# vinodjanardhanan/BatchReactor.jl

Measured on AMD Instinct MI355X. Metric: reactor integrations/sec (CH4 GRI ensemble), higher is better.
Workload: dtype f64

## Files before the change

### batchreactor.jl_amd/_lib.py

```python
import ctypes as C
import os

import numpy as np

HERE = os.path.dirname(os.path.abspath(__file__))
LIBPATH = os.environ.get("BRHIP_LIB") or os.path.join(HERE, "libbrhip.so")

dp = C.POINTER(C.c_double)
ip = C.POINTER(C.c_int)


class MechDesc(C.Structure):
    _fields_ = [
        ("ng", C.c_int), ("ns", C.c_int), ("nrg", C.c_int), ("nrs", C.c_int),
        ("conv", C.c_int), ("p_std", C.c_double),
        ("molwt", dp), ("nasa", dp),
        ("g_nf", ip), ("g_nr", ip), ("g_f", ip), ("g_r", ip), ("g_rev", ip), ("g_tb", ip),
        ("g_arr", dp), ("g_low", dp), ("g_troe_n", ip), ("g_troe", dp), ("g_eff", dp),
        ("site_density", C.c_double), ("sigma", dp),
        ("s_nf", ip), ("s_np", ip), ("s_f", ip), ("s_p", ip), ("s_stick", ip), ("s_arr", dp),
        ("s_ncov", ip), ("s_cov_sp", ip), ("s_cov_eps", dp),
    ]


class Opts(C.Structure):
    _fields_ = [("rtol", C.c_double), ("atol", C.c_double), ("max_steps", C.c_int), ("device", C.c_int),
                ("hmax", C.c_double), ("trace_cap", C.c_int), ("unstable_factor", C.c_double),
                ("ignition_species", C.c_int), ("energy", C.c_int), ("T_end", dp), ("T_out", dp),
                ("nout", C.c_int), ("tout", dp), ("yout", dp),
                ("ntprog", C.c_int), ("tprog_t", dp), ("tprog_T", dp), ("ntprog_rows", C.c_int), ("tprog_row", ip),
                ("dq_jacobian", C.c_int), ("nmult", C.c_int), ("rate_mult", dp), ("rate_mult_row", ip),
                ("tout_per_reactor", C.c_int)]


NSTAT = 20
ENERGY_ADIABATIC_V = 1
BATCH_MAXCOMP = 64


class BatchInput(C.Structure):
    _fields_ = [("gas_mech", C.c_char * 256), ("surface_mech", C.c_char * 256), ("gasphase", C.c_char * 1024),
                ("T", C.c_double), ("p", C.c_double), ("Asv", C.c_double), ("time", C.c_double),
                ("has_T", C.c_int), ("has_p", C.c_int), ("has_Asv", C.c_int), ("has_time", C.c_int),
                ("ncomp", C.c_int), ("comp_is_mass", C.c_int),
                ("comp_names", (C.c_char * 32) * BATCH_MAXCOMP), ("comp_values", C.c_double * BATCH_MAXCOMP)]


EXPORTS = ["br_version", "br_last_error", "br_device_count", "br_mech_create", "br_mech_destroy", "br_mech_info", "br_mech_engine", "br_mech_launch_info",
           "br_rates", "br_rhs", "br_jacobian", "br_integrate", "br_integrate_traced", "br_integrate_multi", "br_integrate_dev",
           "br_last_kernel_ms", "br_debug_lu_solve", "br_mech_parse", "br_host_mech_desc", "br_host_mech_sizes",
           "br_host_mech_species", "br_host_mech_theta0", "br_host_mech_free", "br_mech_compile", "br_read_batch_xml",
           "br_integrate_host", "br_phase_tout_dev", "br_integrate_phase", "br_debug_group_eval",
           "br_debug_group_lu_solve", "br_sensitivity", "br_debug_tprog_eval", "br_debug_lane_eval",
           "br_debug_lane_lu_solve", "br_debug_wave_eval", "br_debug_energy_eval"]

RHS_FN = C.CFUNCTYPE(C.c_int, C.c_void_p, C.c_double, C.POINTER(C.c_double), C.POINTER(C.c_double))
STEP_FN = C.CFUNCTYPE(None, C.c_void_p, C.c_double, C.POINTER(C.c_double))

_lib = None


def lib():
    global _lib
    if _lib is not None:
        return _lib
    if not os.path.exists(LIBPATH):
        raise RuntimeError(f"libbrhip.so not built ({LIBPATH}); run __graft_entry__.build()")
    L = C.CDLL(LIBPATH)
    vp = C.c_void_p
    L.br_version.restype = C.c_int
    L.br_last_error.restype = C.c_char_p
    L.br_device_count.restype = C.c_int
    L.br_mech_create.argtypes = [C.POINTER(MechDesc), C.c_int, C.POINTER(vp)]
    L.br_mech_destroy.argtypes = [vp]
    L.br_mech_info.argtypes = [vp, ip, ip, ip, ip]
    L.br_mech_engine.argtypes = [vp]
    L.br_mech_engine.restype = C.c_int
    L.br_mech_launch_info.argtypes = [vp, ip, ip, C.POINTER(C.c_longlong)]
    L.br_rates.argtypes = [vp, C.c_int, dp, dp, dp, dp, dp, dp]
    L.br_rhs.argtypes = [vp, C.c_int, dp, dp, dp, dp]
    L.br_jacobian.argtypes = [vp, C.c_int, dp, dp, dp, dp]
    L.br_integrate.argtypes = [vp, C.c_int, dp, dp, dp, dp, C.POINTER(Opts), dp]
    L.br_integrate_traced.argtypes = [vp, C.c_int, dp, dp, dp, dp, C.POINTER(Opts), dp, dp]
    L.br_integrate_dev.argtypes = [vp, C.c_int, vp, vp, vp, vp, C.POINTER(Opts), vp, vp]
    L.br_integrate_multi.argtypes = [C.POINTER(vp), C.c_int, C.c_int, dp, dp, dp, dp, C.POINTER(Opts), dp]
    L.br_phase_tout_dev.argtypes = [C.c_int, vp, C.c_int, vp, vp, vp, vp]
    L.br_integrate_phase.argtypes = [vp, C.c_int, dp, dp, dp, dp, C.POINTER(Opts), dp, C.c_int, dp, dp, dp]
    L.br_sensitivity.argtypes = [vp, C.c_int, dp, dp, dp, dp, C.POINTER(Opts), C.c_double, C.c_int, ip, dp, dp, dp, dp,
                                 C.POINTER(C.c_longlong)]
    L.br_last_kernel_ms.argtypes = [vp, dp]
    L.br_debug_lu_solve.argtypes = [C.c_int, C.c_int, dp, dp, dp, dp, ip]
    L.br_debug_lu_solve.restype = C.c_int
    L.br_debug_group_eval.argtypes = [vp, C.c_int, dp, dp, dp, dp, dp]
    L.br_debug_group_eval.restype = C.c_int
    L.br_debug_group_lu_solve.argtypes = [C.c_int, C.c_int, C.c_int, C.c_int, dp, dp, dp, dp, ip, ip]
    L.br_debug_group_lu_solve.restype = C.c_int
    L.br_debug_tprog_eval.argtypes = [C.c_int, C.c_int, dp, dp, C.c_int, ip, C.c_int, dp, dp]
    L.br_debug_tprog_eval.restype = C.c_int
    L.br_debug_lane_eval.argtypes = [vp, C.c_int, dp, dp, C.c_int, dp, ip, dp, dp]
    L.br_debug_lane_eval.restype = C.c_int
    L.br_debug_lane_lu_solve.argtypes = [C.c_int, C.c_int, C.c_int, dp, dp, dp, ip, dp, ip, ip]
    L.br_debug_lane_lu_solve.restype = C.c_int
    L.br_debug_wave_eval.argtypes = [vp, C.c_int, dp, dp, dp, dp, C.c_int, dp, ip, dp, dp]
    L.br_debug_wave_eval.restype = C.c_int
    L.br_debug_energy_eval.argtypes = [vp, C.c_int, dp, dp, C.c_int, dp, ip, dp]
    L.br_debug_energy_eval.restype = C.c_int
    cs = C.c_char_p
    L.br_mech_parse.argtypes = [cs, cs, cs, cs, C.c_int, C.POINTER(vp)]
    L.br_host_mech_desc.argtypes = [vp, C.POINTER(MechDesc)]
    L.br_host_mech_sizes.argtypes = [vp, ip, ip, ip, ip]
    L.br_host_mech_species.argtypes = [vp, C.c_int, C.c_char_p, C.c_size_t]
    L.br_host_mech_theta0.argtypes = [vp, dp]
    L.br_host_mech_free.argtypes = [vp]
    L.br_mech_compile.argtypes = [cs, cs, cs, cs, C.c_int, C.c_int, C.POINTER(vp)]
    L.br_read_batch_xml.argtypes = [cs, C.POINTER(BatchInput)]
    L.br_integrate_host.argtypes = [C.c_int, RHS_FN, vp, dp, C.c_double, C.c_double, C.c_double, C.c_int, STEP_FN, vp,
                                    dp]
    for f in ("br_mech_create", "br_mech_destroy", "br_mech_info", "br_rates", "br_rhs", "br_jacobian",
              "br_integrate", "br_integrate_traced", "br_integrate_multi", "br_integrate_dev", "br_last_kernel_ms",
              "br_mech_parse", "br_host_mech_desc", "br_host_mech_sizes", "br_host_mech_species",
              "br_host_mech_theta0", "br_host_mech_free", "br_mech_compile", "br_read_batch_xml", "br_integrate_host",
              "br_phase_tout_dev", "br_integrate_phase", "br_sensitivity"):
        getattr(L, f).restype = C.c_int
    _lib = L
    return L


def check(rc):
    if rc != 0:
        raise RuntimeError(f"libbrhip error {rc}: {lib().br_last_error().decode()}")


def dptr(a):
    return a.ctypes.data_as(dp) if a is not None else None


def iptr(a):
    return a.ctypes.data_as(ip) if a is not None else None

# ... 31 lines not shown
```

### batchreactor.jl_amd/csrc/brhip_ctl.hpp

```cpp
#pragma once
#include "../../include/brhip.h"
#ifndef BR_ASM_MARKS
#define BR_ASM_MARKS 0
#endif
#ifndef BR_PHASE_CLOCKS
#define BR_PHASE_CLOCKS 0
#endif
#include "brhip_device.hpp"
#if BR_PHASE_CLOCKS
#define BR_CLK_BEGIN                                                                      \
    unsigned long long cyc_rhs = 0, cyc_jac = 0, cyc_lu = 0, cyc_sol = 0, cyc_ctl = 0;    \
    const unsigned long long cyc_all = clock64()
#define BR_CLK_VARS unsigned long long cyc_rhs = 0, cyc_jac = 0, cyc_lu = 0, cyc_sol = 0, cyc_ctl = 0, cyc_all = 0
#define BR_CLK_START() do { cyc_rhs = cyc_jac = cyc_lu = cyc_sol = cyc_ctl = 0; cyc_all = clock64(); } while (0)
#define BR_CLK_STORE(s)                                                                                            \
    do {                                                                                                           \
        (s).cyc_rhs = (double)cyc_rhs; (s).cyc_jac = (double)cyc_jac; (s).cyc_lu = (double)cyc_lu;                 \
        (s).cyc_sol = (double)cyc_sol; (s).cyc_ctl = (double)cyc_ctl; (s).cyc_clk = (double)(clock64() - cyc_all); \
    } while (0)
#define BR_CLK_VALUES (PhaseClk{cyc_rhs, cyc_jac, cyc_lu, cyc_sol, cyc_ctl, cyc_all})
#else
#define BR_CLK_BEGIN
#define BR_CLK_VARS
#define BR_CLK_START()
// ... 790 lines not shown
    if (a.hmax_inv > 0) { const double rh = fabs(h) * a.hmax_inv; if (rh > 1.0) h /= rh; }
    const double tn = ud(C->tn), tstop = ud(C->tstop);
    if ((tn + h - tstop) * h > 0.0) h = (tstop - tn) * (1.0 - 4.0 * UROUND);
    C->h = h; C->hscale = h; C->hprime = h;
    if constexpr (!EN) trace_row<CPL, GW>(C, a, lane, 0, 0.0, z0, z0);
#pragma unroll
    FOR_S V.at(1, s) *= h;
    if (a.max_steps <= 0) { C->status = BR_ERR_MAXSTEPS; return A_DONE; }
    begin_step<CPL, GW>(C, V, lane, a);
    C->phase = PH_NEWTON;
    return A_RHS;
}

__device__ __forceinline__ double root_int(double x, int L) {
    if (L == 1) return x;
    if (L == 2) return sqrt(x);
    if (!(x >= 1e-30 && x <= 1e30)) return pow(x, 1.0 / L);
    double y = (double)__builtin_amdgcn_exp2f(__builtin_amdgcn_logf((float)x) / (float)L);
#pragma unroll
    for (int it = 0; it < 2; ++it) {
        double p = y;
        for (int k = 2; k < L; ++k) p *= y;
        y -= (p * y - x) / (L * p);
    }
    return y;
}
__device__ __forceinline__ double pow_int(double x, int L) {
    double p = x;
    for (int k = 1; k < L; ++k) p *= x;
    return p;
}

template <int CPL, int GW = 64, int VS = GW, bool EN = false>
__device__ BR_CTL_INLINE int ctl_post_solve(LCtl* C, VA<CPL, GW, VS>& V, int lane, double (&delta)[CPL], int lu_fail) {
    BR_SUB_T(ps0);
    BR_QMARK(ps_start);
    const CtlArgs a = load_args<GW>(C);
    const int n = a.n;
    double ewt[CPL], acor[CPL];
#pragma unroll
    FOR_S ewt[s] = V.at(V_EWT, s);
    int nls;
    double acnrm = 0.0;
    const double tq2_e = ud(C->tq[2]);
    if (lu_fail) {
        nls = 2;
    } else {
        C->nni = gui<GW>(C->nni) + 1;
        const double gamrat = ud(C->gamrat);
        const int m = gui<GW>(C->m_it);
        double crate = ud(C->crate);
        const double delp = ud(C->delp), tol = ud(C->tol);
#pragma unroll
        FOR_S {
            if (gamrat != 1.0) delta[s] *= 2.0 / (1.0 + gamrat);
            acor[s] = V.at(V_ACOR, s) + delta[s];
            V.at(V_ACOR, s) = acor[s];
        }
        const double del = wrms_l<CPL, GW>(delta, ewt, lane, n);
        if (m > 0) { crate = fmax(CRDOWN * crate, del / delp); C->crate = crate; }
        const double dcon = del * fmin(1.0, crate) / tol;
        if (dcon <= 1.0) {
            acnrm = (m == 0) ? del : wrms_l<CPL, GW>(acor, ewt, lane, n);
            C->acnrm = acnrm;
            nls = 0;
        } else {
// ... 38 lines not shown
    const int q = gui<GW>(C->q);
    if (dsm > 1.0) {
        const int nef = gui<GW>(C->nef) + 1;
        C->nef = nef; C->netf = gui<GW>(C->netf) + 1;
        cv_restore<CPL, GW>(C, V, lane);
        if (nef == MXNEF) { C->status = BR_ERR_ERRTEST; return A_DONE; }
        C->etamax = 1.0;
        if (nef <= MXNEF1) {
            double eta = 1.0 / (root_int(BIAS2 * dsm, gui<GW>(C->L)) + ADDON);
            eta = fmax(ETAMIN, eta);
            if (nef >= SMALL_NEF) eta = fmin(eta, ETAMXF);
            C->eta = eta;
            cv_rescale<CPL, GW>(C, V, lane);
            begin_attempt<CPL, GW>(C, V, lane, PREV_ERR_FAIL);
            return A_RHS;
        }
        if (q > 1) {
            C->eta = ETAMIN;
            cv_adjust_order<CPL, GW>(C, V, lane, -1);
            C->L = q; C->q = q - 1; C->qwait = q;
            cv_rescale<CPL, GW>(C, V, lane);
            begin_attempt<CPL, GW>(C, V, lane, PREV_ERR_FAIL);
            return A_RHS;
        }
        C->eta = ETAMIN;
        const double h = ud(C->h) * ETAMIN;
        C->h = h; C->hscale = h; C->qwait = LONG_WAIT;
#pragma unroll
        FOR_S V.at(V_Y, s) = V.at(0, s);
        C->phase = PH_EF1;
        return A_RHS;
    }
    BR_SUB_ADD(8, ps0);
    BR_QMARK(ps_complete);
    BR_SUB_T(ps1);
    const int nst = gui<GW>(C->nst) + 1;
    const double h = ud(C->h);
    double tauv[QMAX + 1], lv[QMAX + 1];
#pragma unroll
    for (int i = 1; i <= QMAX; ++i) tauv[i] = ud(C->tau[i]);
#pragma unroll
    for (int j = 0; j <= QMAX; ++j) lv[j] = ud(C->l[j]);
    int qwait = gui<GW>(C->qwait) - 1;
    const double etamax = ud(C->etamax), tq1 = ud(C->tq[1]), tq2 = ud(C->tq[2]), tq3 = ud(C->tq[3]);
    const double tq5 = ud(C->tq[5]);
    double saved_tq5 = ud(C->saved_tq5);
    const int L = gui<GW>(C->L);
    const int nstloc = gui<GW>(C->nstloc) + 1;
    const double tn = ud(C->tn), tstop = ud(C->tstop), ulimit = ud(C->ulimit);
    C->nst = nst;
    double tau2 = tauv[2];
#pragma unroll
    for (int i = QMAX; i >= 2; --i) if (i <= q) C->tau[i] = tauv[i - 1];
    if (q >= 2 || nst > 1) tau2 = tauv[1];
    if ((q == 1) && (nst > 1)) C->tau[2] = tauv[1];
    C->tau[1] = h;
#pragma unroll
    FOR_S acor[s] = V.at(V_ACOR, s);
#pragma unroll
    for (int j = 0; j <= QMAX; ++j) {
        if (j <= q) {
#pragma unroll
            FOR_S V.at(j, s) += lv[j] * acor[s];
        }
    }
    if ((qwait == 1) && (q != QMAX)) {
#pragma unroll
        FOR_S V.at(QMAX, s) = acor[s];
        saved_tq5 = tq5;
        C->saved_tq5 = tq5;
    }
    BR_QMARK(ps_prepare);
    double eta = 1.0, hprime = h;
    int qprime = q;
    if (etamax == 1.0) {
        qwait = qwait > 2 ? qwait : 2;
    } else {
        const int t = lane & 15;
        double xm = 1.0, xp = 1.0;
        bool hm = false, hp = false;
        if (qwait == 0) {
            if (q > 1) {
                double zq[CPL];
#pragma unroll
                FOR_S zq[s] = vget<CPL>(V, q, s);
                const double ddn = wrms_l<CPL, GW>(zq, ewt, lane, n) * tq1;
                xm = BIAS1 * ddn;
                hm = true;
            }
            if (q != QMAX && saved_tq5 != 0.0) {
                const double cquot = (tq5 / saved_tq5) * pow_int(h / tau2, L);
                double tempv[CPL];
#pragma unroll
                FOR_S tempv[s] = acor[s] - cquot * V.at(QMAX, s);
                const double dup = wrms_l<CPL, GW>(tempv, ewt, lane, n) * tq3;
                xp = BIAS3 * dup;
                hp = true;
            }
        }
        const double xa = t == 1 ? xm : (t == 2 ? xp : BIAS2 * dsm);
        const int La = t == 1 ? (hm ? q : L) : (t == 2 ? (hp ? L + 1 : L) : L);
        const double er = 1.0 / (root_int(xa, La) + ADDON);
        const double etaq = row_lane<0>(er);
        BR_XC_AFTER_ETAQ();
        if (qwait != 0) { eta = etaq; }
        else {
            qwait = 2;
            const double etaqm1 = hm ? row_lane<1>(er) : 0.0;
            const double etaqp1 = hp ? row_lane<2>(er) : 0.0;
            const double etam = fmax(etaqm1, fmax(etaq, etaqp1));
            if (etam < THRESH) { eta = 1.0; }
            else if (etam == etaq) { eta = etaq; }
            else if (etam == etaqm1) { eta = etaqm1; qprime = q - 1; }
            else {
                eta = etaqp1; qprime = q + 1;
#pragma unroll
                FOR_S V.at(QMAX, s) = acor[s];
            }
        }
        if (eta < THRESH) { eta = 1.0; hprime = h; }
        else {
            eta = fmin(eta, etamax);
            if (a.hmax_inv > 0) eta /= fmax(1.0, fabs(h) * a.hmax_inv * eta);
            hprime = h * eta;
        }
    }
    C->qwait = qwait;
    C->etamax = (nst <= SMALL_NST) ? ETAMX2 : ETAMX3;
#pragma unroll
    FOR_S V.at(V_ACOR, s) = acor[s] * tq2;
    C->nstloc = nstloc;
    double z0[CPL];
#pragma unroll
    FOR_S z0[s] = V.at(0, s);
    C->eta = eta; C->hprime = hprime; C->qprime = qprime;
    BR_SUB_ADD(9, ps1);
    BR_QMARK(ps_unstable);
    BR_SUB_T(ps2);
    {
        double zm = 0.0;
#pragma unroll
        FOR_S if (CS < n) {
            const double a = fabs(z0[s]);
            if constexpr (EN) zm = fmax(zm, a == a ? (CS == n - 1 && a < INFINITY ? 0.0 : a) : INFINITY);
            else zm = fmax(zm, a == a ? a : INFINITY);
        }
        const double mx = guni<GW>(gmax<GW>(zm));
        if (!(mx < INFINITY) || mx > ulimit) { C->status = BR_ERR_UNSTABLE; return A_DONE; }
    }
    if (!EN && a.trace) {
        double yl[CPL];
#pragma unroll
        FOR_S yl[s] = V.at(V_Y, s);
        trace_row<CPL, GW>(C, a, lane, nst, tn, z0, yl);
    }
    BR_QMARK(ps_ignition);
    if (a.ign >= 0) track_ignition<CPL, GW>(C, a, lane, tn, z0);
    BR_QMARK(ps_dense);
    if (a.nout) dense_output<CPL, GW, VS, EN>(C, V, a, lane, tn, h, q, tn);
    BR_QMARK(ps_tstop);
    const double troundoff = FUZZ * UROUND * (fabs(tn) + fabs(h));
    if (fabs(tn - tstop) <= troundoff) {
        if (a.nout) dense_output<CPL, GW, VS, EN>(C, V, a, lane, tn, h, q, tstop);
        const double sk = (tstop - tn) / h;
#pragma unroll
        FOR_S {
            double yv = vget<CPL>(V, q, s);
#pragma unroll
            for (int j = QMAX - 1; j >= 0; --j) if (j < q) yv = V.at(j, s) + sk * yv;
            V.at(V_Y, s) = yv;
            if (!EN && a.trace && nst <= a.trace_cap) {
                auto row = a.trace + ((size_t)a.rid * (a.trace_cap + 1) + nst) * (2 * n + 4);
                if (lane == 0 && s == 0) row[0] = tstop;
                if (CS < n) row[4 + CS] = yv;
            }
        }
        return A_DONE;
    }
    if ((tn + hprime - tstop) * h > 0.0) {
        hprime = (tstop - tn) * (1.0 - 4.0 * UROUND);
        C->hprime = hprime;
        C->eta = hprime / h;
    }
    if (nstloc >= a.max_steps) { C->status = BR_ERR_MAXSTEPS; return A_DONE; }
    BR_SUB_ADD(10, ps2);
    BR_QMARK(ps_to_begin);
    begin_step<CPL, GW>(C, V, lane, a);
    BR_QMARK(ps_end);
    return A_RHS;
}

constexpr double DQ_SRUR = 1.4901161193847656e-08;
constexpr double DQ_MIN_INC_MULT = 1000.0;
template <int CPL, int GW = 64, int VS = GW>
__device__ __forceinline__ void dq_begin(LCtl* C, VA<CPL, GW, VS>& V, int lane, const double (&f)[CPL]) {
    const int n = gui<GW>(C->a_n);
    double ewt[CPL];
#pragma unroll
    FOR_S {
        ewt[s] = V.at(V_EWT, s);
        V.at(V_TEMP, s) = f[s];
    }
    const double fnorm = wrms_l<CPL, GW>(f, ewt, lane, n);
    C->dq_mininc = (fnorm != 0.0) ? (DQ_MIN_INC_MULT * fabs(ud(C->h)) * UROUND * n * fnorm) : 1.0;
}
template <int CPL, int GW = 64, int VS = GW>
__device__ __forceinline__ void dq_incs(LCtl* C, VA<CPL, GW, VS>& V, int lane, double (&inc)[CPL]) {
    const double mininc = ud(C->dq_mininc);
#pragma unroll
    FOR_S inc[s] = fmax(DQ_SRUR * fabs(V.at(V_Z0, s)), mininc / V.at(V_EWT, s));
}
template <int CPL, int GW = 64, int VS = GW>
__device__ __forceinline__ void dq_column(LCtl* C, VA<CPL, GW, VS>& V, int lane, int j, const double (&f)[CPL], double* Jsave) {
    constexpr int JW = CPL == 2 ? 80 : 64;
    double inc[CPL];
    dq_incs<CPL, GW>(C, V, lane, inc);
    const double ij = (j < 64) ? gbcast<GW>(inc[0], j) : gbcast<GW>(inc[CPL - 1], j - 64);
    const double ii = 1.0 / ij;
    BR_GLOBAL double* col = launder(Jsave) + (size_t)j * JW;
    const int n = gui<GW>(C->a_n);
#pragma unroll
    FOR_S {
// ... 15 lines not shown
```

### batchreactor.jl_amd/csrc/brhip_debug.hpp

```cpp
namespace {
template <int NMAX>
__global__ __launch_bounds__(64) void k_lu_check(int N, int n, const double* J, const double* g, const double* b,
                                                 double* x, double* ws, int* fail) {
    const int rid = blockIdx.x;
    if (rid >= N) return;
    const int lane = threadIdx.x;
    __shared__ double prow[256];
    double* Jt = ws + (size_t)rid * (NMAX * WAVE + lu_ws_doubles(NMAX));
    double* LU = Jt + NMAX * WAVE;
    for (int j = 0; j < NMAX; ++j) Jt[j * WAVE + lane] = (lane < n && j < n) ? J[((size_t)rid * n + lane) * n + j] : 0.0;
    __builtin_amdgcn_fence(__ATOMIC_RELEASE, "workgroup");
    __syncthreads();
    int perm = lane;
    auto factor = [&]() __attribute__((always_inline)) { return lu_factor<NMAX>(Jt, LU, g[rid], n, lane, perm); };
    int f = factor();
    __builtin_amdgcn_fence(__ATOMIC_RELEASE, "workgroup");
    __syncthreads();
    f = factor();
    __builtin_amdgcn_fence(__ATOMIC_RELEASE, "workgroup");
    __syncthreads();
    const double r = lu_solve<NMAX>(LU, n, lane, perm, lane < n ? b[(size_t)rid * n + lane] : 0.0, (LDSd*)prow);
    if (lane < n) x[(size_t)rid * n + lane] = r;
    if (lane == 0) fail[rid] = f;
}
// ... 526 lines not shown
    void* args[] = {(void*)&dm, (void*)&N, (void*)&rpb, (void*)&dT, (void*)&du_, (void*)&ddu, (void*)&dws};
    HIPCHK(hipLaunchKernel(fn, dim3(blocks), dim3(64 * rpb), args, m->e_shmem, 0));
    HIPCHK(hipDeviceSynchronize());
    HIPCHK(hipMemcpy(du, ddu, (size_t)N * (n + 1) * 8, hipMemcpyDeviceToHost));
    return 0;
}

extern "C" int br_debug_tprog_eval(int N, int ntprog, const double* tprog_t, const double* tprog_T, int nrows,
                                   const int* tprog_row, int nt, const double* t, double* Tout) {
    if (N <= 0 || ntprog < 1 || nt < 1 || !t || !Tout) return fail_code_input();
    if (const int rc = check_tprog_arrays(N, ntprog, tprog_t, tprog_T, nrows, tprog_row)) return rc;
    const size_t nk = (size_t)nrows * ntprog, ne = (size_t)N * nt;
    double *dkt, *dkT, *dt, *dTo;
    int* drow = nullptr;
    DevScratch S;
    HIPCHK(S.alloc(&dkt, nk * 8));
    HIPCHK(S.alloc(&dkT, nk * 8));
    HIPCHK(S.alloc(&dt, ne * 8));
    HIPCHK(S.alloc(&dTo, ne * 8));
    HIPCHK(hipMemcpy(dkt, tprog_t, nk * 8, hipMemcpyHostToDevice));
    HIPCHK(hipMemcpy(dkT, tprog_T, nk * 8, hipMemcpyHostToDevice));
    HIPCHK(hipMemcpy(dt, t, ne * 8, hipMemcpyHostToDevice));
    if (tprog_row) {
        HIPCHK(S.alloc(&drow, (size_t)N * 4));
        HIPCHK(hipMemcpy(drow, tprog_row, (size_t)N * 4, hipMemcpyHostToDevice));
    }
    const TProg p{dkt, dkT, drow, ntprog, 0};
    hipLaunchKernelGGL(k_tprog_eval, dim3((N + 63) / 64), dim3(64), 0, 0, N, p, nt, (const double*)dt, dTo);
    HIPCHK(hipGetLastError());
    HIPCHK(hipMemcpy(Tout, dTo, ne * 8, hipMemcpyDeviceToHost));
    return 0;
}

#if BR_PHASE_CLOCKS
extern "C" int br_diag_sub(double* out16) {
    std::vector<unsigned long long> v((size_t)brhip::SUB_MAXW * 16, 0ull);
    if (hipMemcpyFromSymbol(v.data(), HIP_SYMBOL(brhip::g_sub), v.size() * 8) != hipSuccess) return -1;
    for (int i = 0; i < 16; ++i) out16[i] = 0.0;
    for (size_t w = 0; w < (size_t)brhip::SUB_MAXW; ++w)
        for (int i = 0; i < 16; ++i) out16[i] += (double)v[w * 16 + i];
    std::fill(v.begin(), v.end(), 0ull);
    if (hipMemcpyToSymbol(HIP_SYMBOL(brhip::g_sub), v.data(), v.size() * 8) != hipSuccess) return -1;
    return 0;
}
#endif
```

### include/brhip.h

```cpp
#ifndef BRHIP_H
#define BRHIP_H
#include <stddef.h>
#ifdef __cplusplus
extern "C" {
#endif

#define BR_OK             0
#define BR_ERR_MAXSTEPS  -1
#define BR_ERR_ERRTEST   -3
#define BR_ERR_CONV      -4
#define BR_ERR_UNSTABLE  -7
#define BR_ERR_RHS       -8
#define BR_ERR_INPUT    -10
#define BR_ERR_HIP      -20
#define BR_ERR_UNSUPPORTED -30

#define BR_CONV_KC_UNIT_SLIP  1
#define BR_CONV_FALLOFF_XM    2
#define BR_CONV_DOC_COVG      4
#define BR_CONV_TROE_C4      16
#define BR_CONV_REFERENCE    (BR_CONV_KC_UNIT_SLIP | BR_CONV_FALLOFF_XM | BR_CONV_TROE_C4)

#define BR_ENERGY_ADIABATIC_V 1

// ... 130 lines not shown

int br_integrate_phase(br_mech* m, int N, const double* T, const double* Asv, double* u, const double* tf,
                       const br_opts* opts, br_stats* stats, int ntau, const double* tau,
                       double* tout , double* yout );

int br_sensitivity(br_mech* m, int N, const double* T, const double* Asv, const double* u0, const double* tf,
                   const br_opts* opts, double factor, int nsel, const int* rxn ,
                   double* S_tign , double* S_u ,
                   double* u , br_stats* stats ,
                   long long* nbad );

int br_debug_lu_solve(int N, int n, const double* J, const double* gamma, const double* b, double* x, int* fail);

int br_debug_group_eval(br_mech* m, int N, const double* T, const double* Asv, const double* u, double* du, double* J);

int br_debug_group_lu_solve(int gl, int nm, int N, int n, const double* J, const double* gamma, const double* b,
                            double* x, int* fail, int* perm);

int br_debug_lane_eval(br_mech* m, int N, const double* T, const double* u, int nmult, const double* rate_mult,
                       const int* rate_mult_row, double* du, double* J);

int br_debug_lane_lu_solve(int nm, int N, int n, const double* J, const double* gamma, const double* b, const int* skip,
                           double* x, int* fail, int* piv);

int br_debug_wave_eval(br_mech* m, int N, const double* T, const double* Asv, const double* u, const double* T_prev,
                       int nmult, const double* rate_mult, const int* rate_mult_row, double* du, double* J);

int br_debug_energy_eval(br_mech* m, int N, const double* T, const double* u, int nmult, const double* rate_mult,
                         const int* rate_mult_row, double* du );

int br_debug_tprog_eval(int N, int ntprog, const double* tprog_t, const double* tprog_T, int nrows, const int* tprog_row,
                        int nt, const double* t , double* Tout );

typedef int (*br_rhs_fn)(void* user, double t, const double* u, double* du);
typedef void (*br_step_fn)(void* user, double t, const double* u);
int br_integrate_host(int n, br_rhs_fn f, void* user, double* u, double tf, double rtol, double atol, int max_steps,
                      br_step_fn cb, void* cb_user, double* stats);

int br_last_kernel_ms(br_mech* m, double* ms);

#ifdef __cplusplus
}
#endif
#endif
```

Before: 113,000.

## Fuse BDF step completion, order/step selection and next-step setup in registers

```diff
diff --git a/batchreactor.jl_amd/_lib.py b/batchreactor.jl_amd/_lib.py
--- a/batchreactor.jl_amd/_lib.py
+++ b/batchreactor.jl_amd/_lib.py
@@ -52,7 +52,7 @@
            "br_host_mech_species", "br_host_mech_theta0", "br_host_mech_free", "br_mech_compile", "br_read_batch_xml",
            "br_integrate_host", "br_phase_tout_dev", "br_integrate_phase", "br_debug_group_eval",
            "br_debug_group_lu_solve", "br_sensitivity", "br_debug_tprog_eval", "br_debug_lane_eval",
-           "br_debug_lane_lu_solve", "br_debug_wave_eval", "br_debug_energy_eval"]
+           "br_debug_lane_lu_solve", "br_debug_wave_eval", "br_debug_energy_eval", "br_debug_step_boundary"]
 
 RHS_FN = C.CFUNCTYPE(C.c_int, C.c_void_p, C.c_double, C.POINTER(C.c_double), C.POINTER(C.c_double))
 STEP_FN = C.CFUNCTYPE(None, C.c_void_p, C.c_double, C.POINTER(C.c_double))
@@ -105,6 +105,8 @@
     L.br_debug_wave_eval.restype = C.c_int
     L.br_debug_energy_eval.argtypes = [vp, C.c_int, dp, dp, C.c_int, dp, ip, dp]
     L.br_debug_energy_eval.restype = C.c_int
+    L.br_debug_step_boundary.argtypes = [C.c_int, C.c_int, C.c_int, vp, dp, vp, dp, ip]
+    L.br_debug_step_boundary.restype = C.c_int
     cs = C.c_char_p
     L.br_mech_parse.argtypes = [cs, cs, cs, cs, C.c_int, C.POINTER(vp)]
     L.br_host_mech_desc.argtypes = [vp, C.POINTER(MechDesc)]
diff --git a/batchreactor.jl_amd/csrc/brhip_ctl.hpp b/batchreactor.jl_amd/csrc/brhip_ctl.hpp
--- a/batchreactor.jl_amd/csrc/brhip_ctl.hpp
+++ b/batchreactor.jl_amd/csrc/brhip_ctl.hpp
@@ -846,6 +846,406 @@
 }
 
 template <int CPL, int GW = 64, int VS = GW, bool EN = false>
+__device__ __forceinline__ int step_tail_plain(LCtl* C, VA<CPL, GW, VS>& V, int lane, const CtlArgs& a, const double (&z0)[CPL],
+                                               int nst, double tn, double h, int q, double tstop, double hprime, int nstloc) {
+    const int n = a.n;
+    BR_SUB_T(pt0);
+    if (!EN && a.trace) {
+        double yl[CPL];
+#pragma unroll
+        FOR_S yl[s] = V.at(V_Y, s);
+        trace_row<CPL, GW>(C, a, lane, nst, tn, z0, yl);
+    }
+    BR_QMARK(ps_ignition);
+    if (a.ign >= 0) track_ignition<CPL, GW>(C, a, lane, tn, z0);
+    BR_QMARK(ps_dense);
+    if (a.nout) dense_output<CPL, GW, VS, EN>(C, V, a, lane, tn, h, q, tn);
+    BR_QMARK(ps_tstop);
+    const double troundoff = FUZZ * UROUND * (fabs(tn) + fabs(h));
+    if (fabs(tn - tstop) <= troundoff) {
+        if (a.nout) dense_output<CPL, GW, VS, EN>(C, V, a, lane, tn, h, q, tstop);
+        const double sk = (tstop - tn) / h;
+#pragma unroll
+        FOR_S {
+            double yv = vget<CPL>(V, q, s);
+#pragma unroll
+            for (int j = QMAX - 1; j >= 0; --j) if (j < q) yv = V.at(j, s) + sk * yv;
+            V.at(V_Y, s) = yv;
+            if (!EN && a.trace && nst <= a.trace_cap) {
+                auto row = a.trace + ((size_t)a.rid * (a.trace_cap + 1) + nst) * (2 * n + 4);
+                if (lane == 0 && s == 0) row[0] = tstop;
+                if (CS < n) row[4 + CS] = yv;
+            }
+        }
+        return A_DONE;
+    }
+    if ((tn + hprime - tstop) * h > 0.0) {
+        hprime = (tstop - tn) * (1.0 - 4.0 * UROUND);
+        C->hprime = hprime;
+        C->eta = hprime / h;
+    }
+    if (nstloc >= a.max_steps) { C->status = BR_ERR_MAXSTEPS; return A_DONE; }
+    BR_SUB_ADD(10, pt0);
+    BR_QMARK(ps_to_begin);
+    begin_step<CPL, GW>(C, V, lane, a);
+    BR_QMARK(ps_end);
+    return A_RHS;
+}
+
+template <int CPL, int GW = 64, int VS = GW, bool EN = false>
+__device__ __forceinline__ int step_boundary_plain(LCtl* C, VA<CPL, GW, VS>& V, int lane, const CtlArgs& a,
+                                                   const double (&ewt)[CPL], double dsm, int q) {
+    const int n = a.n;
+    double acor[CPL];
+    BR_QMARK(ps_complete);
+    BR_SUB_T(ps1);
+    const int nst = gui<GW>(C->nst) + 1;
+    const double h = ud(C->h);
+    double tauv[QMAX + 1], lv[QMAX + 1];
+#pragma unroll
+    for (int i = 1; i <= QMAX; ++i) tauv[i] = ud(C->tau[i]);
+#pragma unroll
+    for (int j = 0; j <= QMAX; ++j) lv[j] = ud(C->l[j]);
+    int qwait = gui<GW>(C->qwait) - 1;
+    const double etamax = ud(C->etamax), tq1 = ud(C->tq[1]), tq2 = ud(C->tq[2]), tq3 = ud(C->tq[3]);
+    const double tq5 = ud(C->tq[5]);
+    double saved_tq5 = ud(C->saved_tq5);
+    const int L = gui<GW>(C->L);
+    const int nstloc = gui<GW>(C->nstloc) + 1;
+    const double tn = ud(C->tn), tstop = ud(C->tstop), ulimit = ud(C->ulimit);
+    C->nst = nst;
+    double tau2 = tauv[2];
+#pragma unroll
+    for (int i = QMAX; i >= 2; --i) if (i <= q) C->tau[i] = tauv[i - 1];
+    if (q >= 2 || nst > 1) tau2 = tauv[1];
+    if ((q == 1) && (nst > 1)) C->tau[2] = tauv[1];
+    C->tau[1] = h;
+#pragma unroll
+    FOR_S acor[s] = V.at(V_ACOR, s);
+#pragma unroll
+    for (int j = 0; j <= QMAX; ++j) {
+        if (j <= q) {
+#pragma unroll
+            FOR_S V.at(j, s) += lv[j] * acor[s];
+        }
+    }
+    if ((qwait == 1) && (q != QMAX)) {
+#pragma unroll
+        FOR_S V.at(QMAX, s) = acor[s];
+        saved_tq5 = tq5;
+        C->saved_tq5 = tq5;
+    }
+    BR_QMARK(ps_prepare);
+    double eta = 1.0, hprime = h;
+    int qprime = q;
+    if (etamax == 1.0) {
+        qwait = qwait > 2 ? qwait : 2;
+    } else {
+        const int t = lane & 15;
+        double xm = 1.0, xp = 1.0;
+        bool hm = false, hp = false;
+        if (qwait == 0) {
+            if (q > 1) {
+                double zq[CPL];
+#pragma unroll
+                FOR_S zq[s] = vget<CPL>(V, q, s);
+                const double ddn = wrms_l<CPL, GW>(zq, ewt, lane, n) * tq1;
+                xm = BIAS1 * ddn;
+                hm = true;
+            }
+            if (q != QMAX && saved_tq5 != 0.0) {
+                const double cquot = (tq5 / saved_tq5) * pow_int(h / tau2, L);
+                double tempv[CPL];
+#pragma unroll
+                FOR_S tempv[s] = acor[s] - cquot * V.at(QMAX, s);
+                const double dup = wrms_l<CPL, GW>(tempv, ewt, lane, n) * tq3;
+                xp = BIAS3 * dup;
+                hp = true;
+            }
+        }
+        const double xa = t == 1 ? xm : (t == 2 ? xp : BIAS2 * dsm);
+        const int La = t == 1 ? (hm ? q : L) : (t == 2 ? (hp ? L + 1 : L) : L);
+        const double er = 1.0 / (root_int(xa, La) + ADDON);
+        const double etaq = row_lane<0>(er);
+        BR_XC_AFTER_ETAQ();
+        if (qwait != 0) { eta = etaq; }
+        else {
+            qwait = 2;
+            const double etaqm1 = hm ? row_lane<1>(er) : 0.0;
+            const double etaqp1 = hp ? row_lane<2>(er) : 0.0;
+            const double etam = fmax(etaqm1, fmax(etaq, etaqp1));
+            if (etam < THRESH) { eta = 1.0; }
+            else if (etam == etaq) { eta = etaq; }
+            else if (etam == etaqm1) { eta = etaqm1; qprime = q - 1; }
+            else {
+                eta = etaqp1; qprime = q + 1;
+#pragma unroll
+                FOR_S V.at(QMAX, s) = acor[s];
+            }
+        }
+        if (eta < THRESH) { eta = 1.0; hprime = h; }
+        else {
+            eta = fmin(eta, etamax);
+            if (a.hmax_inv > 0) eta /= fmax(1.0, fabs(h) * a.hmax_inv * eta);
+            hprime = h * eta;
+        }
+    }
+    C->qwait = qwait;
+    C->etamax = (nst <= SMALL_NST) ? ETAMX2 : ETAMX3;
+#pragma unroll
+    FOR_S V.at(V_ACOR, s) = acor[s] * tq2;
+    C->nstloc = nstloc;
+    double z0[CPL];
+#pragma unroll
+    FOR_S z0[s] = V.at(0, s);
+    C->eta = eta; C->hprime = hprime; C->qprime = qprime;
+    BR_SUB_ADD(9, ps1);
+    BR_QMARK(ps_unstable);
+    BR_SUB_T(ps2);
+    {
+        double zm = 0.0;
+#pragma unroll
+        FOR_S if (CS < n) {
+            const double a = fabs(z0[s]);
+            if constexpr (EN) zm = fmax(zm, a == a ? (CS == n - 1 && a < INFINITY ? 0.0 : a) : INFINITY);
+            else zm = fmax(zm, a == a ? a : INFINITY);
+        }
+        const double mx = guni<GW>(gmax<GW>(zm));
+        if (!(mx < INFINITY) || mx > ulimit) { C->status = BR_ERR_UNSTABLE; return A_DONE; }
+    }
+    BR_SUB_ADD(10, ps2);
+    return step_tail_plain<CPL, GW, VS, EN>(C, V, lane, a, z0, nst, tn, h, q, tstop, hprime, nstloc);
+}
+
+#ifndef BR_STEP_FUSED
+#define BR_STEP_FUSED 1
+#endif
+__device__ __forceinline__ void opaque_v(double& x) { asm volatile("" : "+v"(x)); }
+template <int CPL, int GW = 64, int VS = GW, bool EN = false>
+__device__ __forceinline__ int step_boundary_fused(LCtl* C, VA<CPL, GW, VS>& V, int lane, const CtlArgs& a,
+                                                   const double (&ewt)[CPL], double dsm, int q) {
+    static_assert(GW == 64, "step_boundary_fused: the wavefront engine's form");
+    const int n = a.n;
+    BR_SUB_T(ps1);
+    const int nst = gui<GW>(C->nst) + 1;
+    const double h = ud(C->h), hscale = ud(C->hscale);
+    double tauv[QMAX + 1], lv[QMAX + 1];
+#pragma unroll
+    for (int i = 1; i <= QMAX; ++i) tauv[i] = ud(C->tau[i]);
+#pragma unroll
+    for (int j = 0; j <= QMAX; ++j) lv[j] = ud(C->l[j]);
+    int qwait = gui<GW>(C->qwait) - 1;
+    const double etamax = ud(C->etamax), tq1 = ud(C->tq[1]), tq2 = ud(C->tq[2]), tq3 = ud(C->tq[3]);
+    const double tq5 = ud(C->tq[5]);
+    double saved_tq5 = ud(C->saved_tq5);
+    const int L = gui<GW>(C->L);
+    const int nstloc = gui<GW>(C->nstloc) + 1;
+    const double tn = ud(C->tn), tstop = ud(C->tstop), ulimit = ud(C->ulimit);
+    double acor[CPL], z[QMAX + 1][CPL];
+#pragma unroll
+    FOR_S {
+        acor[s] = V.at(V_ACOR, s);
+#pragma unroll
+        for (int j = 0; j <= QMAX; ++j) z[j][s] = V.at(j, s);
+    }
+    auto opaque_z = [&]() {
+#pragma unroll
+        FOR_S {
+#pragma unroll
+            for (int j = 0; j <= QMAX; ++j) opaque_v(z[j][s]);
+        }
+    };
+    auto store_completed = [&]() {
+#pragma unroll
+        FOR_S {
+#pragma unroll
+            for (int j = 0; j <= QMAX; ++j) V.at(j, s) = z[j][s];
+            V.at(V_ACOR, s) = acor[s] * tq2;
+        }
+    };
+    C->nst = nst;
+    double tau2 = tauv[2];
+#pragma unroll
+    for (int i = QMAX; i >= 2; --i) if (i <= q) C->tau[i] = tauv[i - 1];
+    if (q >= 2 || nst > 1) tau2 = tauv[1];
+    if ((q == 1) && (nst > 1)) C->tau[2] = tauv[1];
+    C->tau[1] = h;
+#pragma unroll
+    for (int j = 0; j <= QMAX; ++j) {
+        if (j <= q) {
+#pragma unroll
+            FOR_S z[j][s] += lv[j] * acor[s];
+        }
+    }
+    opaque_z();
+    if ((qwait == 1) && (q != QMAX)) {
+#pragma unroll
+        FOR_S z[QMAX][s] = acor[s];
+        saved_tq5 = tq5;
+        C->saved_tq5 = tq5;
+    }
+    double eta = 1.0, hprime = h;
+    int qprime = q;
+    if (etamax == 1.0) {
+        qwait = qwait > 2 ? qwait : 2;
+    } else {
+        const int t = lane & 15;
+        double xm = 1.0, xp = 1.0;
+        bool hm = false, hp = false;
+        if (qwait == 0) {
+            if (q > 1) {
+                double zq[CPL];
+#pragma unroll
+                FOR_S {
+                    double r = 0.0;
+#pragma unroll
+                    for (int jj = 0; jj <= QMAX; ++jj) if (jj == q) r = z[jj][s];
+                    zq[s] = r;
+                }
+                const double ddn = wrms_l<CPL, GW>(zq, ewt, lane, n) * tq1;
+                xm = BIAS1 * ddn;
+                hm = true;
+            }
+            if (q != QMAX && saved_tq5 != 0.0) {
+                const double cquot = (tq5 / saved_tq5) * pow_int(h / tau2, L);
+                double tempv[CPL];
+#pragma unroll
+                FOR_S tempv[s] = acor[s] - cquot * z[QMAX][s];
+                const double dup = wrms_l<CPL, GW>(tempv, ewt, lane, n) * tq3;
+                xp = BIAS3 * dup;
+                hp = true;
+            }
+        }
+        const double xa = t == 1 ? xm : (t == 2 ? xp : BIAS2 * dsm);
+        const int La = t == 1 ? (hm ? q : L) : (t == 2 ? (hp ? L + 1 : L) : L);
+        const double er = 1.0 / (root_int(xa, La) + ADDON);
+        const double etaq = row_lane<0>(er);
+        BR_XC_AFTER_ETAQ();
+        if (qwait != 0) { eta = etaq; }
+        else {
+            qwait = 2;
+            const double etaqm1 = hm ? row_lane<1>(er) : 0.0;
+            const double etaqp1 = hp ? row_lane<2>(er) : 0.0;
+            const double etam = fmax(etaqm1, fmax(etaq, etaqp1));
+            if (etam < THRESH) { eta = 1.0; }
+            else if (etam == etaq) { eta = etaq; }
+            else if (etam == etaqm1) { eta = etaqm1; qprime = q - 1; }
+            else {
+                eta = etaqp1; qprime = q + 1;
+#pragma unroll
+                FOR_S z[QMAX][s] = acor[s];
+            }
+        }
+        if (eta < THRESH) { eta = 1.0; hprime = h; }
+        else {
+            eta = fmin(eta, etamax);
+            if (a.hmax_inv > 0) eta /= fmax(1.0, fabs(h) * a.hmax_inv * eta);
+            hprime = h * eta;
+        }
+    }
+    C->qwait = qwait;
+    C->etamax = (nst <= SMALL_NST) ? ETAMX2 : ETAMX3;
+    C->nstloc = nstloc;
+    double z0[CPL];
+#pragma unroll
+    FOR_S z0[s] = z[0][s];
+    C->eta = eta; C->hprime = hprime; C->qprime = qprime;
+    BR_SUB_ADD(9, ps1);
+    BR_SUB_T(ps2);
+    {
+        double zm = 0.0;
+#pragma unroll
+        FOR_S if (CS < n) {
+            const double a = fabs(z0[s]);
+            if constexpr (EN) zm = fmax(zm, a == a ? (CS == n - 1 && a < INFINITY ? 0.0 : a) : INFINITY);
+            else zm = fmax(zm, a == a ? a : INFINITY);
+        }
+        const double mx = guni<GW>(gmax<GW>(zm));
+        if (!(mx < INFINITY) || mx > ulimit) { store_completed(); C->status = BR_ERR_UNSTABLE; return A_DONE; }
+    }
+    const double troundoff = FUZZ * UROUND * (fabs(tn) + fabs(h));
+    if ((!EN && a.trace) || a.nout || fabs(tn - tstop) <= troundoff || nstloc >= a.max_steps) {
+        store_completed();
+        BR_SUB_ADD(10, ps2);
+        return step_tail_plain<CPL, GW, VS, EN>(C, V, lane, a, z0, nst, tn, h, q, tstop, hprime, nstloc);
+    }
+    if (a.ign >= 0) track_ignition<CPL, GW>(C, a, lane, tn, z0);
+    if ((tn + hprime - tstop) * h > 0.0) {
+        hprime = (tstop - tn) * (1.0 - 4.0 * UROUND);
+        C->hprime = hprime;
+        eta = hprime / h;
+        C->eta = eta;
+    }
+    BR_SUB_ADD(10, ps2);
+    BR_SUB_T(bt0);
+#pragma unroll
+    FOR_S V.at(V_EWT, s) = (CS < a.n) ? 1.0 / (a.rtol * fabs(z0[s]) + a.atol) : 1.0;
+    C->saved_t = tn;
+    C->ncf = 0; C->nef = 0;
+    if (hprime != h) {
+        int qn = q;
+        if (qprime != q) {
+#pragma unroll
+            FOR_S {
+#pragma unroll
+                for (int j = 0; j <= QMAX; ++j) V.at(j, s) = z[j][s];
+            }
+            cv_adjust_order<CPL, GW>(C, V, lane, qprime - q);
+            C->q = qprime; C->L = qprime + 1; C->qwait = qprime + 1;
+#pragma unroll
+            FOR_S {
+#pragma unroll
+                for (int j = 0; j <= QMAX; ++j) z[j][s] = V.at(j, s);
+            }
+            qn = qprime;
+        }
+        double f = eta;
+#pragma unroll
+        for (int j = 1; j <= QMAX; ++j) {
+            if (j <= qn) {
+#pragma unroll
+                FOR_S z[j][s] *= f;
+                f *= eta;
+            }
+        }
+        opaque_z();
+        const double hn = hscale * eta;
+        C->h = hn; C->hscale = hn;
+    }
+    const AttemptIn in = load_attempt<GW>(C);
+    {
+        double tp = in.tn + in.h;
+        if ((tp - in.tstop) * in.h > 0) tp = in.tstop;
+        C->tn = tp;
+#pragma unroll
+        FOR_S {
+#pragma unroll
+            for (int k = 1; k <= QMAX; ++k)
+#pragma unroll
+                for (int j = QMAX; j >= k; --j)
+                    if (j <= in.q && k <= in.q) z[j - 1][s] += z[j][s];
+#pragma unroll
+            for (int j = 0; j <= QMAX; ++j) V.at(j, s) = z[j][s];
+        }
+    }
+    double tq4, gamrat;
+    cv_set_lp(C, in, tq4, gamrat);
+    BR_XC_AFTER_CVSET();
+    C->convfail = NO_FAILURES;
+    C->callSetup = (in.nst == 0) || (in.nst >= in.nstlp + MSBP) || (fabs(gamrat - 1.0) > DGMAX);
+#pragma unroll
+    FOR_S V.at(V_ACOR, s) = 0.0;
+    C->tol = tq4;
+    C->jbad = 0;
+    C->jcur_nls = 0;
+    C->m_it = 0;
+#pragma unroll
+    FOR_S V.at(V_Y, s) = z[0][s];
+    BR_SUB_ADD(7, bt0);
+    return A_RHS;
+}
+
+template <int CPL, int GW = 64, int VS = GW, bool EN = false>
 __device__ BR_CTL_INLINE int ctl_post_solve(LCtl* C, VA<CPL, GW, VS>& V, int lane, double (&delta)[CPL], int lu_fail) {
     BR_SUB_T(ps0);
     BR_QMARK(ps_start);
@@ -950,162 +1350,8 @@
         return A_RHS;
     }
     BR_SUB_ADD(8, ps0);
-    BR_QMARK(ps_complete);
-    BR_SUB_T(ps1);
-    const int nst = gui<GW>(C->nst) + 1;
-    const double h = ud(C->h);
-    double tauv[QMAX + 1], lv[QMAX + 1];
-#pragma unroll
-    for (int i = 1; i <= QMAX; ++i) tauv[i] = ud(C->tau[i]);
-#pragma unroll
-    for (int j = 0; j <= QMAX; ++j) lv[j] = ud(C->l[j]);
-    int qwait = gui<GW>(C->qwait) - 1;
-    const double etamax = ud(C->etamax), tq1 = ud(C->tq[1]), tq2 = ud(C->tq[2]), tq3 = ud(C->tq[3]);
-    const double tq5 = ud(C->tq[5]);
-    double saved_tq5 = ud(C->saved_tq5);
-    const int L = gui<GW>(C->L);
-    const int nstloc = gui<GW>(C->nstloc) + 1;
-    const double tn = ud(C->tn), tstop = ud(C->tstop), ulimit = ud(C->ulimit);
-    C->nst = nst;
-    double tau2 = tauv[2];
-#pragma unroll
-    for (int i = QMAX; i >= 2; --i) if (i <= q) C->tau[i] = tauv[i - 1];
-    if (q >= 2 || nst > 1) tau2 = tauv[1];
-    if ((q == 1) && (nst > 1)) C->tau[2] = tauv[1];
-    C->tau[1] = h;
-#pragma unroll
-    FOR_S acor[s] = V.at(V_ACOR, s);
-#pragma unroll
-    for (int j = 0; j <= QMAX; ++j) {
-        if (j <= q) {
-#pragma unroll
-            FOR_S V.at(j, s) += lv[j] * acor[s];
-        }
-    }
-    if ((qwait == 1) && (q != QMAX)) {
-#pragma unroll
-        FOR_S V.at(QMAX, s) = acor[s];
-        saved_tq5 = tq5;
-        C->saved_tq5 = tq5;
-    }
-    BR_QMARK(ps_prepare);
-    double eta = 1.0, hprime = h;
-    int qprime = q;
-    if (etamax == 1.0) {
-        qwait = qwait > 2 ? qwait : 2;
-    } else {
-        const int t = lane & 15;
-        double xm = 1.0, xp = 1.0;
-        bool hm = false, hp = false;
-        if (qwait == 0) {
-            if (q > 1) {
-                double zq[CPL];
-#pragma unroll
-                FOR_S zq[s] = vget<CPL>(V, q, s);
-                const double ddn = wrms_l<CPL, GW>(zq, ewt, lane, n) * tq1;
-                xm = BIAS1 * ddn;
-                hm = true;
-            }
-            if (q != QMAX && saved_tq5 != 0.0) {
-                const double cquot = (tq5 / saved_tq5) * pow_int(h / tau2, L);
-                double tempv[CPL];
-#pragma unroll
-                FOR_S tempv[s] = acor[s] - cquot * V.at(QMAX, s);
-                const double dup = wrms_l<CPL, GW>(tempv, ewt, lane, n) * tq3;
-                xp = BIAS3 * dup;
-                hp = true;
-            }
-        }
-        const double xa = t == 1 ? xm : (t == 2 ? xp : BIAS2 * dsm);
-        const int La = t == 1 ? (hm ? q : L) : (t == 2 ? (hp ? L + 1 : L) : L);
-        const double er = 1.0 / (root_int(xa, La) + ADDON);
-        const double etaq = row_lane<0>(er);
-        BR_XC_AFTER_ETAQ();
-        if (qwait != 0) { eta = etaq; }
-        else {
-            qwait = 2;
-            const double etaqm1 = hm ? row_lane<1>(er) : 0.0;
-            const double etaqp1 = hp ? row_lane<2>(er) : 0.0;
-            const double etam = fmax(etaqm1, fmax(etaq, etaqp1));
-            if (etam < THRESH) { eta = 1.0; }
-            else if (etam == etaq) { eta = etaq; }
-            else if (etam == etaqm1) { eta = etaqm1; qprime = q - 1; }
-            else {
-                eta = etaqp1; qprime = q + 1;
-#pragma unroll
-                FOR_S V.at(QMAX, s) = acor[s];
-            }
-        }
-        if (eta < THRESH) { eta = 1.0; hprime = h; }
-        else {
-            eta = fmin(eta, etamax);
-            if (a.hmax_inv > 0) eta /= fmax(1.0, fabs(h) * a.hmax_inv * eta);
-            hprime = h * eta;
-        }
-    }
-    C->qwait = qwait;
-    C->etamax = (nst <= SMALL_NST) ? ETAMX2 : ETAMX3;
-#pragma unroll
-    FOR_S V.at(V_ACOR, s) = acor[s] * tq2;
-    C->nstloc = nstloc;
-    double z0[CPL];
-#pragma unroll
-    FOR_S z0[s] = V.at(0, s);
-    C->eta = eta; C->hprime = hprime; C->qprime = qprime;
-    BR_SUB_ADD(9, ps1);
-    BR_QMARK(ps_unstable);
-    BR_SUB_T(ps2);
-    {
-        double zm = 0.0;
-#pragma unroll
-        FOR_S if (CS < n) {
-            const double a = fabs(z0[s]);
-            if constexpr (EN) zm = fmax(zm, a == a ? (CS == n - 1 && a < INFINITY ? 0.0 : a) : INFINITY);
-            else zm = fmax(zm, a == a ? a : INFINITY);
-        }
-        const double mx = guni<GW>(gmax<GW>(zm));
-        if (!(mx < INFINITY) || mx > ulimit) { C->status = BR_ERR_UNSTABLE; return A_DONE; }
-    }
-    if (!EN && a.trace) {
-        double yl[CPL];
-#pragma unroll
-        FOR_S yl[s] = V.at(V_Y, s);
-        trace_row<CPL, GW>(C, a, lane, nst, tn, z0, yl);
-    }
-    BR_QMARK(ps_ignition);
-    if (a.ign >= 0) track_ignition<CPL, GW>(C, a, lane, tn, z0);
-    BR_QMARK(ps_dense);
-    if (a.nout) dense_output<CPL, GW, VS, EN>(C, V, a, lane, tn, h, q, tn);
-    BR_QMARK(ps_tstop);
-    const double troundoff = FUZZ * UROUND * (fabs(tn) + fabs(h));
-    if (fabs(tn - tstop) <= troundoff) {
-        if (a.nout) dense_output<CPL, GW, VS, EN>(C, V, a, lane, tn, h, q, tstop);
-        const double sk = (tstop - tn) / h;
-#pragma unroll
-        FOR_S {
-            double yv = vget<CPL>(V, q, s);
-#pragma unroll
-            for (int j = QMAX - 1; j >= 0; --j) if (j < q) yv = V.at(j, s) + sk * yv;
-            V.at(V_Y, s) = yv;
-            if (!EN && a.trace && nst <= a.trace_cap) {
-                auto row = a.trace + ((size_t)a.rid * (a.trace_cap + 1) + nst) * (2 * n + 4);
-                if (lane == 0 && s == 0) row[0] = tstop;
-                if (CS < n) row[4 + CS] = yv;
-            }
-        }
-        return A_DONE;
-    }
-    if ((tn + hprime - tstop) * h > 0.0) {
-        hprime = (tstop - tn) * (1.0 - 4.0 * UROUND);
-        C->hprime = hprime;
-        C->eta = hprime / h;
-    }
-    if (nstloc >= a.max_steps) { C->status = BR_ERR_MAXSTEPS; return A_DONE; }
-    BR_SUB_ADD(10, ps2);
-    BR_QMARK(ps_to_begin);
-    begin_step<CPL, GW>(C, V, lane, a);
-    BR_QMARK(ps_end);
-    return A_RHS;
+    if constexpr (BR_STEP_FUSED && GW == 64 && VS == GW) return step_boundary_fused<CPL, GW, VS, EN>(C, V, lane, a, ewt, dsm, q);
+    else return step_boundary_plain<CPL, GW, VS, EN>(C, V, lane, a, ewt, dsm, q);
 }
 
 constexpr double DQ_SRUR = 1.4901161193847656e-08;
diff --git a/batchreactor.jl_amd/csrc/brhip_debug.hpp b/batchreactor.jl_amd/csrc/brhip_debug.hpp
--- a/batchreactor.jl_amd/csrc/brhip_debug.hpp
+++ b/batchreactor.jl_amd/csrc/brhip_debug.hpp
@@ -582,6 +582,115 @@
     return 0;
 }
 
+namespace {
+template <int NMAX, bool FUSED>
+__global__ __launch_bounds__(256) void k_step_boundary(int N, int nwaves, const char* ctl, const double* vec, char* ctl_out,
+                                                       double* vec_out, int* code) {
+    constexpr int CPL = NMAX > 64 ? 2 : 1;
+    constexpr int VS = vec_stride(NMAX);
+    constexpr int W = CPL == 2 ? 72 : 64;
+    constexpr int RB = CTL_BYTES + (CPL == 2 ? (V1OFF + 8 * (NVEC - 1) + 72 + 64) * 8 : NVEC * VS * 8);
+    extern __shared__ __attribute__((aligned(16))) char smem_raw[];
+    const int wave = uni((int)(threadIdx.x >> 6)), lane = threadIdx.x & 63;
+    const size_t roff = (size_t)wave * RB;
+    LCtl* C = (LCtl*)(smem_raw + roff);
+    typedef __attribute__((address_space(3))) unsigned LU32;
+    LU32* cw = (LU32*)(smem_raw + roff);
+    VA<CPL, 64, VS> V{(LDbl*)(smem_raw + roff + CTL_BYTES), lane};
+    for (int i = blockIdx.x * 4 + wave; i < N; i += nwaves) {
+        const unsigned* src = reinterpret_cast<const unsigned*>(ctl + (size_t)i * CTL_BYTES);
+        for (int k = lane; k < CTL_BYTES / 4; k += 64) cw[k] = src[k];
+#pragma unroll
+        FOR_S {
+            const int c = CS;
+#pragma unroll
+            for (int j = 0; j < NVEC; ++j) V.at(j, s) = c < W ? vec[((size_t)i * NVEC + j) * W + c] : 0.0;
+        }
+        wave_sync();
+        double ewt[CPL];
+#pragma unroll
+        FOR_S ewt[s] = V.at(V_EWT, s);
+        const CtlArgs a = load_args<64>(C);
+        const int q = ui(C->q);
+        const double dsm = ud(C->acnrm) * ud(C->tq[2]);
+        int act;
+        if constexpr (FUSED) act = step_boundary_fused<CPL, 64, VS, false>(C, V, lane, a, ewt, dsm, q);
+        else act = step_boundary_plain<CPL, 64, VS, false>(C, V, lane, a, ewt, dsm, q);
+        wave_sync();
+        unsigned* dst = reinterpret_cast<unsigned*>(ctl_out + (size_t)i * CTL_BYTES);
+        for (int k = lane; k < CTL_BYTES / 4; k += 64) dst[k] = cw[k];
+#pragma unroll
+        FOR_S {
+            const int c = CS;
+            const bool real = CPL == 2 ? c < W : lane < VS;
+#pragma unroll
+            for (int j = 0; j < NVEC; ++j) {
+                const double x = V.at(j, s);
+                if (real) vec_out[((size_t)i * NVEC + j) * W + c] = x;
+            }
+        }
+        if (lane == 0) code[i] = act;
+        wave_sync();
+    }
+}
+template <bool FUSED>
+const void* step_boundary_kernel(int nmax) {
+    return nmax == 16 ? (const void*)k_step_boundary<16, FUSED> : nmax == 32 ? (const void*)k_step_boundary<32, FUSED>
+         : nmax == 56 ? (const void*)k_step_boundary<56, FUSED> : nmax == 64 ? (const void*)k_step_boundary<64, FUSED>
+                                                                              : (const void*)k_step_boundary<72, FUSED>;
+}
+}
+
+extern "C" int br_debug_step_boundary(int n, int N, int ctl_bytes, const void* ctl, const double* vec, void* ctl_out,
+                                      double* vec_out, int* code_out) {
+    if (n <= 0 || n > 72 || N <= 0 || !ctl || !vec || !ctl_out || !vec_out || !code_out) return fail_code_input();
+    if (ctl_bytes != CTL_BYTES) return fail(BR_ERR_INPUT, "br_debug_step_boundary: not this library's controller block size");
+    const int nmax = nmax_of(n), cpl = nmax > 64 ? 2 : 1, W = cpl == 2 ? 72 : 64;
+    std::vector<char> hc((size_t)N * CTL_BYTES);
+    memcpy(hc.data(), ctl, hc.size());
+    for (int i = 0; i < N; ++i) {
+        Ctl c;
+        memcpy(&c, hc.data() + (size_t)i * CTL_BYTES, sizeof(Ctl));
+        if (c.q < 1 || c.q > QMAX || c.L != c.q + 1 || c.a_n != n)
+            return fail(BR_ERR_INPUT, "br_debug_step_boundary: block with q outside 1..5, L != q + 1 or a_n != n");
+        c.a_trace = nullptr; c.a_tout = nullptr; c.a_yout = nullptr;
+        c.a_nout = 0; c.a_trace_cap = 0; c.a_ign = -1; c.iout = 0;
+        memcpy(hc.data() + (size_t)i * CTL_BYTES, &c, sizeof(Ctl));
+    }
+    const size_t cb = (size_t)N * CTL_BYTES, vb = (size_t)N * NVEC * W * 8;
+    char *dc, *dco;
+    double *dv, *dvo;
+    int* dcode;
+    DevScratch S;
+    HIPCHK(S.alloc(&dc, cb));
+    HIPCHK(S.alloc(&dv, vb));
+    HIPCHK(S.alloc(&dco, 2 * cb));
+    HIPCHK(S.alloc(&dvo, 2 * vb));
+    HIPCHK(S.alloc(&dcode, (size_t)2 * N * 4));
+    HIPCHK(hipMemcpy(dc, hc.data(), cb, hipMemcpyHostToDevice));
+    HIPCHK(hipMemcpy(dv, vec, vb, hipMemcpyHostToDevice));
+    HIPCHK(hipMemset(dco, 0, 2 * cb));
+    HIPCHK(hipMemset(dvo, 0, 2 * vb));
+    HIPCHK(hipMemset(dcode, 0, (size_t)2 * N * 4));
+    const int blocks = std::max(1, std::min(64, N / 8));
+    const int nwaves = blocks * 4;
+    const int shmem = 4 * (CTL_BYTES + vec_bytes(cpl, vec_stride(nmax)));
+    for (int f = 0; f < 2; ++f) {
+        const void* fn = f ? step_boundary_kernel<true>(nmax) : step_boundary_kernel<false>(nmax);
+        char* oc = dco + (size_t)f * cb;
+        double* ov = dvo + (size_t)f * N * NVEC * W;
+        int* ocode = dcode + (size_t)f * N;
+        int Nn = N, nw = nwaves;
+        void* args[] = {(void*)&Nn, (void*)&nw, (void*)&dc, (void*)&dv, (void*)&oc, (void*)&ov, (void*)&ocode};
+        HIPCHK(hipLaunchKernel(fn, dim3(blocks), dim3(256), args, shmem, 0));
+    }
+    HIPCHK(hipDeviceSynchronize());
+    HIPCHK(hipMemcpy(ctl_out, dco, 2 * cb, hipMemcpyDeviceToHost));
+    HIPCHK(hipMemcpy(vec_out, dvo, 2 * vb, hipMemcpyDeviceToHost));
+    HIPCHK(hipMemcpy(code_out, dcode, (size_t)2 * N * 4, hipMemcpyDeviceToHost));
+    return 0;
+}
+
 #if BR_PHASE_CLOCKS
 extern "C" int br_diag_sub(double* out16) {
     std::vector<unsigned long long> v((size_t)brhip::SUB_MAXW * 16, 0ull);
diff --git a/batchreactor.jl_amd/stepcheck.py b/batchreactor.jl_amd/stepcheck.py
--- /dev/null
+++ b/batchreactor.jl_amd/stepcheck.py
@@ -0,0 +1,68 @@
+import ctypes as C
+
+import numpy as np
+
+from . import _lib
+
+QMAX = 5
+NVEC = 10
+V_ACOR, V_EWT, V_TEMP, V_Y = 6, 7, 8, 9
+A_RHS, A_SOLVE, A_SETUP, A_DONE = 0, 1, 2, 3
+
+
+class CtlBlock(C.Structure):
+    _fields_ = (
+        [("p_last", C.c_double), ("tau", C.c_double * (QMAX + 2)), ("tq", C.c_double * 6), ("l", C.c_double * (QMAX + 1))]
+        + [(k, C.c_double) for k in ("tn", "h", "rl1", "gamma", "gamrat", "gammap", "crate", "delp", "hprime", "hscale",
+                                     "eta", "etamax", "acnrm", "saved_tq5", "saved_t", "tol", "hg", "hub", "hlb", "hnew",
+                                     "ulimit", "tstop")]
+        + [(k, C.c_int) for k in ("q", "qprime", "L", "qwait", "nst", "nfe", "nsetups", "nje", "nni", "ncfn", "netf",
+                                  "nstlp", "nstlj", "ncf", "nef", "nstloc", "status", "m_it", "convfail", "count1",
+                                  "phase", "callSetup", "jbad", "jcur_nls", "hnewOK", "newj")]
+        + [(k, C.c_double) for k in ("ign_x", "ign_t", "ign_rate", "t_ign", "ign_dt", "dq_mininc")]
+        + [("nfe_dq", C.c_int), ("iout", C.c_int)]
+        + [(k, C.c_double) for k in ("a_rtol", "a_atol", "a_hmax_inv", "a_ufac")]
+        + [(k, C.c_void_p) for k in ("a_trace", "a_tout", "a_yout")]
+        + [(k, C.c_int) for k in ("a_max_steps", "a_trace_cap", "a_rid", "a_n", "a_ign", "a_nout")])
+
+
+CTL_BYTES = (C.sizeof(CtlBlock) + 15) // 16 * 16
+CTL_DTYPE = np.dtype((np.void, CTL_BYTES))
+
+
+def vec_width(n):
+    return 72 if n > 64 else 64
+
+
+def pack_ctl(blocks):
+    out = np.zeros((len(blocks), CTL_BYTES), dtype=np.uint8)
+    for i, b in enumerate(blocks):
+        out[i, :C.sizeof(CtlBlock)] = np.frombuffer(bytes(b), dtype=np.uint8)
+    return out
+
+
+def unpack_ctl(row):
+    return CtlBlock.from_buffer_copy(np.ascontiguousarray(row).tobytes()[:C.sizeof(CtlBlock)])
+
+
+def step_boundary(n, ctl, vec):
+    if not isinstance(n, (int, np.integer)) or not 1 <= n <= 72:
+        raise ValueError(f"n = {n!r}: 1 .. 72")
+    ctl = np.asarray(ctl)
+    vec = np.asarray(vec)
+    if ctl.dtype != np.uint8 or ctl.ndim != 2 or ctl.shape[1] != CTL_BYTES:
+        raise ValueError(f"ctl: uint8 [N][{CTL_BYTES}], got {ctl.dtype} {ctl.shape}")
+    N = ctl.shape[0]
+    if N < 1:
+        raise ValueError("ctl: no states")
+    W = vec_width(int(n))
+    if vec.dtype != np.float64 or vec.shape != (N, NVEC, W):
+        raise ValueError(f"vec: float64 [{N}][{NVEC}][{W}], got {vec.dtype} {vec.shape}")
+    ctl = np.ascontiguousarray(ctl)
+    vec = np.ascontiguousarray(vec)
+    ctl_out = np.zeros((2, N, CTL_BYTES), dtype=np.uint8)
+    vec_out = np.zeros((2, N, NVEC, W), dtype=np.float64)
+    code = np.zeros((2, N), dtype=np.int32)
+    _lib.check(_lib.lib().br_debug_step_boundary(int(n), N, CTL_BYTES, ctl.ctypes.data_as(C.c_void_p), _lib.dptr(vec),
+                                                 ctl_out.ctypes.data_as(C.c_void_p), _lib.dptr(vec_out), _lib.iptr(code)))
+    return ctl_out, vec_out, code
diff --git a/include/brhip.h b/include/brhip.h
--- a/include/brhip.h
+++ b/include/brhip.h
@@ -186,6 +186,9 @@
 int br_debug_tprog_eval(int N, int ntprog, const double* tprog_t, const double* tprog_T, int nrows, const int* tprog_row,
                         int nt, const double* t , double* Tout );
 
+int br_debug_step_boundary(int n, int N, int ctl_bytes, const void* ctl, const double* vec, void* ctl_out, double* vec_out,
+                           int* code_out);
+
 typedef int (*br_rhs_fn)(void* user, double t, const double* u, double* du);
 typedef void (*br_step_fn)(void* user, double t, const double* u);
 int br_integrate_host(int n, br_rhs_fn f, void* user, double* u, double tf, double rtol, double atol, int max_steps,
```

Result: no change. 113,700, median of 6 (+0.6%).
